# luoyetx/JDA

Measured on AMD Instinct MI355X. Metric: candidate windows/sec, 640x480 batch (jdaDetect hot path); FDDB images/sec in config.fddb_images_per_s, higher is better.
Workload: dtype f32

## Files before the change

### jda_amd/csrc/host.h

```cpp
#pragma once
#include <hip/hip_runtime_api.h>

#include <algorithm>
#include <atomic>
#include <chrono>
#include <cmath>
#include <cstdio>
#include <cstdlib>
#include <cstring>
#include <condition_variable>
#include <exception>
#include <functional>
#include <memory>
#include <map>
#include <mutex>
#include <numeric>
#include <new>
#include <stdexcept>
#include <string>
#include <thread>
#include <tuple>
#include <vector>

#include "../../include/jda.h"
// ... 34 lines not shown
  catch (const std::exception& e) { std::snprintf(buf, sizeof buf, "%s", e.what()); what = buf; }
  catch (...) {}
  try { fail(std::string(fn) + ": " + what); }
  catch (...) { std::fprintf(stderr, "libjda: %s: %s\n", fn, what); }
  if (sync_device) { (void)hipDeviceSynchronize(); (void)hipGetLastError(); }
}
#define JDA_ABI_CATCH(ret) catch (...) { jda::abi_exception(__func__, false); return ret; }
#define JDA_ABI_CATCH_SYNC(ret) catch (...) { jda::abi_exception(__func__, true); return ret; }
#define JDA_ABI_CATCH_VOID catch (...) { jda::abi_exception(__func__, false); }

constexpr int kLdsGranule = 1280, kLdsGranules = 128;
inline int lds_wgs_per_cu(long long lds_bytes) { return lds_bytes <= 0 ? kLdsGranules : (int)(kLdsGranules / ((lds_bytes + kLdsGranule - 1) / kLdsGranule)); }
inline int lds_bytes_for_wgs(int wgs_per_cu) { return (kLdsGranules / std::max(1, wgs_per_cu)) * kLdsGranule; }

inline long long env_ll(const char* name, long long dflt) {
  const char* v = std::getenv(name);
  return v && *v ? std::atoll(v) : dflt;
}

#define JDA_KNOBS(X)                                                                                   \
  X(handoff, "JDA_HANDOFF", 128)             \
  X(no_fast_scan, "JDA_NO_FAST_SCAN", 0)                                                               \
  X(plan_cache, "JDA_PLAN_CACHE", 64)                                 \
  X(dense, "JDA_DENSE", 1)                                                \
  X(merge_blocks, "JDA_MERGE_BLOCKS", 2048)  \
  X(side_small, "JDA_SIDE_SMALL", 1)                                                                   \
  X(side_stream, "JDA_SIDE_STREAM", 1)                                                                 \
  X(wide_max, "JDA_WIDE_MAX", 1024)          \
  X(wide_conc, "JDA_WIDE_CONC", 1)           \
  X(h2d_stream, "JDA_H2D_STREAM", 1)         \
  X(h2d_min_bytes, "JDA_H2D_MIN_BYTES", 8 << 20)  \
  X(kernel_d2h, "JDA_KERNEL_D2H", 1)         \
  X(filter0, "JDA_FILTER0", 1)               \
  X(predict, "JDA_PREDICT", 1)               \
  X(debug_times, "JDA_DEBUG_TIMES", 0)                                                                 \
  X(test_wpf_scale, "JDA_TEST_WPF_SCALE", 1)              \
  X(test_throw, "JDA_TEST_THROW", 0)         \
  X(lanes, "JDA_LANES", 2)                                 \
  X(lanes_min_windows, "JDA_LANES_MIN_WINDOWS", 2000000)                                               \
  X(workspace_mb, "JDA_WORKSPACE_MB", 24 * 1024)                                                       \
  X(ws_bound, "JDA_WS_BOUND", 1)             \
  X(ws_factor_pct, "JDA_WS_FACTOR_PCT", 400)  \
  X(ws_min_entries, "JDA_WS_MIN_ENTRIES", 65536)  \
  X(ragged_chunk_windows, "JDA_RAGGED_CHUNK_WINDOWS", 4000000)  \
  X(ragged_chunk_windows_cpp, "JDA_RAGGED_CHUNK_WINDOWS_CPP", 8000000)  \
  X(mine_chunk_windows, "JDA_MINE_CHUNK_WINDOWS", 4194304)  \
  X(ragged_chunk_min_windows, "JDA_RAGGED_CHUNK_MIN_WINDOWS", 1500000)  \
  X(ragged_split, "JDA_RAGGED_SPLIT", 3)     \
  X(ragged_single_windows, "JDA_RAGGED_SINGLE_WINDOWS", 5000000)  \
  X(hwq_place, "JDA_HWQ_PLACE", 1)           \
  X(max_lanes, "JDA_MAX_LANES", 16)          \
  X(lane_idle_calls, "JDA_LANE_IDLE_CALLS", 256)  \
  X(device_post, "JDA_DEVICE_POST", 1)       \
  X(device_post_min_frames, "JDA_DEVICE_POST_MIN_FRAMES", 16)  \
  X(w_pad, "JDA_W_PAD", 1)                   \
  X(lm_deep, "JDA_LM_DEEP", 1)               \
  X(w_stream_mb, "JDA_W_STREAM_MB", 8)       \
  X(scan_p, "JDA_SCAN_P", 1)                 \
  X(scan_p_ragged, "JDA_SCAN_P_RAGGED", 1)   \
  X(scan_p_block, "JDA_SCAN_P_BLOCK", 768)                               \
  X(scan_p_slots, "JDA_SCAN_P_SLOTS", 5)     \
  X(scan_p_b0, "JDA_SCAN_P_B0", 32)                \
  X(scan_p_b1, "JDA_SCAN_P_B1", 64)                                                                    \
  X(scan_p_b2, "JDA_SCAN_P_B2", 0)                                                                     \
  X(scan_p_b3, "JDA_SCAN_P_B3", 0)                                                                     \
  X(scan_p_b4, "JDA_SCAN_P_B4", 0)                                                                     \
// ... 454 lines not shown
```

### jda_amd/csrc/k_finish.hip

```cpp
#include "finish_common.h"

#ifndef FIN_ROW_BATCH
#define FIN_ROW_BATCH 0
#endif

namespace jda {


template <typename DL, bool TRACE, int kG, bool MULTI, bool ST, bool STREAM = false>
__global__ __launch_bounds__(64) void k_finish(const DevPlan* __restrict__ plan, DevModelT<typename DL::Real> m,
                                               WorkT<typename DL::Real> w, int multi_i, float inv_sqrt2,
                                               int t_begin, int t_end, int apply_th, typename DL::Real final_th,
                                               const S0Node* __restrict__ s0_table, int tile_win, int survivors) {
  using Real = typename DL::Real;
  constexpr bool kCpp = sizeof(Real) == 8;
  extern __shared__ __attribute__((aligned(16))) unsigned char lds[];
  const int lane = threadIdx.x;
  const int T = m.T, K = m.K, node_n = m.node_n, leaf_n = m.leaf_n, dim = m.dim, w_pitch = m.w_pitch;
  const int dim_pad = (dim + 1) & ~1;
  Real* sh = (Real*)lds;
  uint32_t* lbf = (uint32_t*)(sh + dim_pad);
  int* stage_cnt = (int*)(lbf + ((K + 3) & ~3));
  Real* st_tmp = (Real*)(stage_cnt + kMaxStages);
  uint8_t* tile = lds + (((size_t)((unsigned char*)(st_tmp + (ST ? 2 * dim_pad + 8 : 0)) - lds) + 15) & ~(size_t)15);
  constexpr bool multi = MULTI;
  (void)multi_i;
  if (lane < kMaxStages) stage_cnt[lane] = 0;
  const bool from_scan = t_begin == 0 && !survivors;
  const unsigned n = (unsigned)min(w.counters[from_scan ? kCntTail : kCntMid], (unsigned long long)(from_scan ? w.cap_q : w.cap_m));
  unsigned long long carts_acc = 0;

#ifdef JDA_SCAN_TIMING
  unsigned long long stamps[15];
  int n_stamp = 0;
  int dbg_win = 0;
#define JDA_FSTAMP() do { if (n_stamp < 15) stamps[n_stamp++] = __builtin_amdgcn_s_memtime(); } while (0)
#else
#define JDA_FSTAMP() do { } while (0)
#endif
  for (unsigned i = blockIdx.x; i < n; i += gridDim.x) {
    JDA_FSTAMP();
    const uint32_t gid = from_scan ? w.q_gid[i] : w.m_gid[i];
    Real score = from_scan ? w.q_score[i] : w.m_score[i];
    const int kstart = from_scan ? (int)w.q_kstart[i] : (survivors ? K : 0);
    unsigned hash = kFnvSeed;
    if (TRACE) hash = from_scan ? w.q_hash[i] : w.m_hash[i];
    int win;
    View v0{}, v1{}, v2{};
    const uint32_t xy = from_scan ? w.q_xy[i] : w.m_xy[i];
    const uint32_t wf = from_scan ? w.q_wf[i] : w.m_wf[i];
    decode_window<Real>(plan, w, xy, wf, inv_sqrt2, &win, &v0, &v1, &v2, multi);
    const S0Node* s0_tbl = nullptr;
    if (!MULTI && s0_table != nullptr && t_begin == 0) {
      const bool hit = lane < plan->n_levels && plan->lv[lane].win == win;
      const unsigned long long mh = __ballot(hit);
      if (mh) {
        const DevLevel lv = plan->lv[__ffsll((long long)mh) - 1];
        if (lv.tiled) s0_tbl = s0_table + lv.s0_table;
      }
    }
    const uint8_t* wbase = v0.img + (size_t)v0.oy * v0.w + v0.ox;
#ifdef JDA_SCAN_TIMING
    dbg_win = win;
#endif
    const bool use_tile = !MULTI && win <= tile_win;
    const int tpitch = (win + 3) & ~3;
    __syncthreads();
    if (!MULTI && use_tile) load_window_tile(wbase, v0.w, win, tile, tpitch, lane, 64, v0.bc);
    {
      const Real* src = t_begin == 0 ? m.mean_shape : w.m_shape + (size_t)i * dim;
      for (int d = lane; d < dim; d += 64) sh[d] = src[d];
    }
    __syncthreads();
    JDA_FSTAMP();

    bool alive = true;
    int carts_n = 0;
    for (int t = t_begin; t < t_end; t++) {
      const NodeOff<Real>* n_off = (const NodeOff<Real>*)m.lm_off + (size_t)t * K * node_n;
      const uint2* n_meta = m.lm_meta + (size_t)t * K * node_n;
      const int n_split = m.lm_split;
      const typename DL::Node* n_deep = (const typename DL::Node*)m.lm_deep + (size_t)t * K * (node_n - ((1 << min(n_split, m.D - 1)) - 1));
      const Real* leaf_tab = m.leaf + (size_t)t * K * leaf_n;
      const Real* cth = m.cth + (size_t)t * K;
      const Real* cmean = m.cmean + (size_t)t * K;
      const Real* cstd = m.cstd + (size_t)t * K;
      const uint8_t* cnorm = m.cnorm + (size_t)t * K;
      const int kbeg = t == 0 ? min(kstart, K) : 0;
      const int k_first = kbeg & ~63;
      Stp<Real> stp;
      stp.scale = 1; stp.r00 = 1; stp.r01 = 0; stp.r10 = 0; stp.r11 = 1;
      if constexpr (ST) {
        const bool stale = t == m.similarity - 2;
        if (lane == 0 && (!stale || t == t_begin)) {
          Stp<double> p;
          p.scale = 1.; p.r00 = 1.; p.r01 = 0.; p.r10 = 0.; p.r11 = 1.;
          if (!stale) p = stp_calc((const double*)sh, (const double*)m.mean_shape_raw, m.L, (double*)st_tmp, (double*)st_tmp + dim_pad);
          double* o = (double*)st_tmp + 2 * dim_pad;
          o[0] = p.scale; o[1] = p.r00; o[2] = p.r01; o[3] = p.r10; o[4] = p.r11;
        }
        __syncthreads();
        const Real* o = st_tmp + 2 * dim_pad;
        stp.scale = o[0]; stp.r00 = o[1]; stp.r01 = o[2]; stp.r10 = o[3]; stp.r11 = o[4];
      }
      const bool apply_st = ST && t > 0;

      for (int k0 = k_first; k0 < K && alive; k0 += 64 * kG) {
        int kk[kG], lf[kG], nrm[kG];
        Real ls[kG], thk[kG], mk[kG], sk[kG];
#pragma unroll
        for (int g = 0; g < kG; g++) kk[g] = min(k0 + g * 64 + lane, K - 1);
        if (t == 0 && s0_tbl && use_tile) walk_carts_s0<kG, true>(s0_tbl, K, kk, m.D, node_n, tile, tpitch, lf, Bc(0, (long long)tpitch * win));
        else if (t == 0 && s0_tbl) walk_carts_s0<kG, false>(s0_tbl, K, kk, m.D, node_n, wbase, v0.w, lf, v0.bc);
        else if (!MULTI && use_tile) walk_carts<DL, kG, MULTI, ST, true>(n_off, n_meta, K, kk, m.D, node_n, sh, win, v0, v1, v2, stp, apply_st, lf, tile, tpitch, n_deep, n_split);
        else walk_carts<DL, kG, MULTI, ST>(n_off, n_meta, K, kk, m.D, node_n, sh, win, v0, v1, v2, stp, apply_st, lf, nullptr, 0, n_deep, n_split);
#pragma unroll
        for (int g = 0; g < kG; g++) {
          const int k = k0 + g * 64 + lane;
          ls[g] = 0; thk[g] = 0; mk[g] = 0; sk[g] = 1; nrm[g] = 0;
          if (k < K) {
            lbf[k] = (uint32_t)(k * leaf_n + lf[g]) * (uint32_t)w_pitch;
            ls[g] = leaf_tab[(unsigned)(k * leaf_n + lf[g])];
            thk[g] = cth[k];
            nrm[g] = cnorm[k];
            if (nrm[g]) { mk[g] = cmean[k]; sk[g] = cstd[k]; }
          }
        }
#pragma unroll
        for (int g = 0; g < kG; g++) {
          const int kg = k0 + g * 64;
          if (kg >= K || !alive) break;
          const unsigned long long normmask = __ballot(nrm[g] != 0);
          const int jr = replay_scores<Real, TRACE>(score, hash, ls[g], thk[g], mk[g], sk[g], normmask, lf[g],
                                                    max(0, kbeg - kg), min(64, K - kg));
          if (jr >= 0) { alive = false; carts_n = t * K + kg + jr + 1; }
        }
        if (t == t_begin) JDA_FSTAMP();
      }
      if (t != t_begin) JDA_FSTAMP();
      if (!alive) break;
      for (int k0 = 0; k0 < k_first; k0 += 128) {
        int kk[2], lf[2];
        kk[0] = min(k0 + lane, k_first - 1); kk[1] = min(k0 + 64 + lane, k_first - 1);
        if (t == 0 && s0_tbl && use_tile) walk_carts_s0<2, true>(s0_tbl, K, kk, m.D, node_n, tile, tpitch, lf, Bc(0, (long long)tpitch * win));
        else if (t == 0 && s0_tbl) walk_carts_s0<2, false>(s0_tbl, K, kk, m.D, node_n, wbase, v0.w, lf, v0.bc);
        else if (!MULTI && use_tile) walk_carts<DL, 2, MULTI, ST, true>(n_off, n_meta, K, kk, m.D, node_n, sh, win, v0, v1, v2, stp, apply_st, lf, tile, tpitch, n_deep, n_split);
        else walk_carts<DL, 2, MULTI, ST>(n_off, n_meta, K, kk, m.D, node_n, sh, win, v0, v1, v2, stp, apply_st, lf, nullptr, 0, n_deep, n_split);
        if (k0 + lane < k_first) lbf[k0 + lane] = (uint32_t)((k0 + lane) * leaf_n + lf[0]) * (uint32_t)w_pitch;
        if (k0 + 64 + lane < k_first) lbf[k0 + 64 + lane] = (uint32_t)((k0 + 64 + lane) * leaf_n + lf[1]) * (uint32_t)w_pitch;
      }
      __syncthreads();
      if (t == t_begin) JDA_FSTAMP();
      const Real* wt = m.w_rows + (size_t)t * K * leaf_n * w_pitch;
      for (int d = lane; d < dim; d += 64) {
        Real acc = kCpp ? (Real)0 : sh[d];
        const Real* col = wt + d;
        int k = 0;
#ifdef JDA_EXP_NOREG
        k = K;
#endif
        constexpr int RB = FIN_ROW_BATCH > 0 ? FIN_ROW_BATCH : (kCpp ? 32 : 64);
        for (; k + RB <= K; k += RB) {
          Real r[RB];
#pragma unroll
          for (int u = 0; u < RB; u++) { JDA_BC(Bc(0, (long long)K * leaf_n * w_pitch), (long long)lbf[k + u] + d, 1, kBcWRow); r[u] = STREAM ? __builtin_nontemporal_load(col + lbf[k + u]) : col[lbf[k + u]]; }
#pragma unroll
          for (int u = 0; u < RB; u++) acc = acc + r[u];
        }
        for (; k < K; k++) { JDA_BC(Bc(0, (long long)K * leaf_n * w_pitch), (long long)lbf[k] + d, 1, kBcWRow); acc = acc + col[lbf[k]]; }
        if (kCpp) {
          const Real other = __shfl_xor(acc, 1);
          acc = (d & 1) ? stp.scale * (stp.r10 * other + stp.r11 * acc) : stp.scale * (stp.r00 * acc + stp.r01 * other);
          acc = sh[d] + acc;
// ... 49 lines not shown
namespace {
__device__ __forceinline__ int walk_cart_s0_d4(const S0Node* __restrict__ tbl, unsigned K, unsigned k,
                                               const uint8_t* __restrict__ pix, int pitch, const Bc& bc = Bc()) {
  const S0Node r0 = tbl[k];
  const uint4 c1 = *(const uint4*)(tbl + K + 2u * k);
  const uint4 c2a = *(const uint4*)(tbl + 3u * K + 4u * k);
  const uint4 c2b = *(const uint4*)(tbl + 3u * K + 4u * k + 2u);
  auto left = [&](uint32_t lo, uint32_t hi) {
    const unsigned p1 = lo & 0x3fffffu, p2 = __builtin_amdgcn_alignbit(hi, lo, 22) & 0x3fffffu;
    JDA_BC_ADDR(bc, pix + __umul24(p1 >> 11, (unsigned)pitch) + (p1 & 0x7ffu), 1, kBcFinishPix);
    JDA_BC_ADDR(bc, pix + __umul24(p2 >> 11, (unsigned)pitch) + (p2 & 0x7ffu), 1, kBcFinishPix);
    const int a = pix[__umul24(p1 >> 11, (unsigned)pitch) + (p1 & 0x7ffu)];
    const int b = pix[__umul24(p2 >> 11, (unsigned)pitch) + (p2 & 0x7ffu)];
    return a - b <= (int)((hi >> 12) & 0x3ffu) - 256;
  };
  const bool l0 = left(r0.lo, r0.hi);
  const uint32_t lo1 = l0 ? c1.x : c1.z, hi1 = l0 ? c1.y : c1.w;
  const bool l1 = left(lo1, hi1);
  const uint32_t lo2 = l0 ? (l1 ? c2a.x : c2a.z) : (l1 ? c2b.x : c2b.z);
  const uint32_t hi2 = l0 ? (l1 ? c2a.y : c2a.w) : (l1 ? c2b.y : c2b.w);
  const bool l2 = left(lo2, hi2);
  const int n1 = l0 ? 1 : 2, n2 = 2 * n1 + (l1 ? 1 : 2), n3 = 2 * n2 + (l2 ? 1 : 2);
  return n3 - 7;
}
}

template <typename DL, bool TRACE>
__global__ __launch_bounds__(256) void k_filter0(const DevPlan* __restrict__ plan, DevModelT<typename DL::Real> m,
                                                 WorkT<typename DL::Real> w, const S0Node* __restrict__ s0_table) {
  using Real = typename DL::Real;
  constexpr int NW = 2;
  const int lane = threadIdx.x & 63, wv = threadIdx.x >> 6;
  const int K = m.K, node_n = m.node_n, leaf_n = m.leaf_n;
  const unsigned n = (unsigned)min(w.counters[kCntTail], (unsigned long long)w.cap_q);
  const Real* leaf_tab = m.leaf;
  const int W = plan->width;
#ifdef JDA_BOUNDS_CHECK
  const Bc bc_fr((long long)(uintptr_t)w.bc_lo, (long long)(uintptr_t)w.bc_hi);
#else
  const Bc bc_fr;
#endif
  unsigned long long carts_acc = 0;
  const unsigned waves = gridDim.x * 4u;
  for (unsigned i0 = blockIdx.x * 4u + (unsigned)wv; i0 < n; i0 += NW * waves) {
    unsigned idx[NW]; bool has[NW];
    uint32_t gid[NW], xy[NW], wf[NW];
    Real score[NW];
    int kbeg[NW], rej[NW];
    unsigned hash[NW];
    const uint8_t* wbase[NW];
    const S0Node* tbl[NW];
#pragma unroll
    for (int u = 0; u < NW; u++) {
      idx[u] = i0 + (unsigned)u * waves; has[u] = idx[u] < n;
      const unsigned i = has[u] ? idx[u] : i0;
      gid[u] = w.q_gid[i]; score[u] = w.q_score[i]; kbeg[u] = min((int)w.q_kstart[i], K);
      hash[u] = TRACE ? w.q_hash[i] : kFnvSeed;
      xy[u] = w.q_xy[i]; wf[u] = w.q_wf[i];
      rej[u] = has[u] ? -1 : 0;
    }
#pragma unroll
    for (int u = 0; u < NW; u++) {
      const int win = (int)(wf[u] & 0xffffu), frame = (int)(wf[u] >> 16);
      const uint8_t* img = w.img_off != nullptr ? w.frames + w.img_off[frame] : w.frames + (size_t)frame * w.frame_stride;
      wbase[u] = img + (size_t)(xy[u] >> 16) * W + (xy[u] & 0xffffu);
      tbl[u] = s0_table;
      const bool hit = lane < plan->n_levels && plan->lv[lane].win == win;
      const unsigned long long mh = __ballot(hit);
      if (mh) tbl[u] = s0_table + plan->lv[__ffsll((long long)mh) - 1].s0_table;
    }
    int k0[NW];
#pragma unroll
    for (int u = 0; u < NW; u++) k0[u] = kbeg[u] & ~63;
    for (;;) {
      bool go[NW], any = false;
#pragma unroll
      for (int u = 0; u < NW; u++) { go[u] = rej[u] < 0 && k0[u] < K; any = any || go[u]; }
      if (!any) break;
      int lf[NW], nrm[NW];
      Real ls[NW], thk[NW], mk[NW], sk[NW];
#pragma unroll
      for (int u = 0; u < NW; u++) {
        const int k = k0[u] + lane;
        thk[u] = 0; nrm[u] = 0; ls[u] = 0; mk[u] = 0; sk[u] = 1; lf[u] = 0;
        if (go[u] && k < K) { thk[u] = m.cth[k]; nrm[u] = m.cnorm[k]; }
      }
#pragma unroll
      for (int u = 0; u < NW; u++) {
        if (!go[u]) continue;
        int kk[1], l1[1];
        kk[0] = min(k0[u] + lane, K - 1);
        if (m.D == 4) l1[0] = walk_cart_s0_d4(tbl[u], (unsigned)K, (unsigned)kk[0], wbase[u], W, bc_fr);
        else walk_carts_s0<1, false>(tbl[u], K, kk, m.D, node_n, wbase[u], W, l1, bc_fr);
        lf[u] = l1[0];
      }
#pragma unroll
      for (int u = 0; u < NW; u++) {
        const int k = k0[u] + lane;
        if (go[u] && k < K) {
          ls[u] = leaf_tab[(unsigned)(k * leaf_n + lf[u])];
          if (nrm[u]) { mk[u] = m.cmean[k]; sk[u] = m.cstd[k]; }
        }
      }
#pragma unroll
      for (int u = 0; u < NW; u++) {
        if (!go[u]) continue;
        const unsigned long long normmask = __ballot(nrm[u] != 0);
        const int jr = replay_scores<Real, TRACE>(score[u], hash[u], ls[u], thk[u], mk[u], sk[u], normmask, lf[u],
                                                  max(0, kbeg[u] - k0[u]), min(64, K - k0[u]));
        if (jr >= 0) rej[u] = k0[u] + jr;
        k0[u] += 64;
      }
    }
#pragma unroll
    for (int u = 0; u < NW; u++) {
      if (!has[u]) continue;
      if (rej[u] >= 0) {
        carts_acc += (unsigned long long)(rej[u] + 1);
        if (TRACE && lane == 0) { w.tr_carts[gid[u]] = rej[u] + 1; w.tr_score[gid[u]] = score[u]; w.tr_hash[gid[u]] = hash[u]; }
      } else {
        unsigned o = 0;
        if (lane == 0) o = (unsigned)atomicAdd(&w.counters[kCntMid], 1ull);
        o = (unsigned)__shfl((int)o, 0);
        if (o < w.cap_m && lane == 0) {
          w.m_gid[o] = gid[u]; w.m_score[o] = score[u]; w.m_xy[o] = xy[u]; w.m_wf[o] = wf[u];
          if (TRACE) w.m_hash[o] = hash[u];
        }
      }
    }
  }
  if (lane == 0 && carts_acc) atomicAdd(shard_counter(w.counters, kCntCarts), carts_acc);
}

template <typename Real>
hipError_t launch_filter0(bool trace, const DevPlan* d_plan, const DevModelT<Real>& m, const WorkT<Real>& w, long long n_hint,
                          const S0Node* s0_table, hipStream_t stream) {
  using DL = typename std::conditional<sizeof(Real) == 4, DialectC, DialectCPP>::type;
  const unsigned blocks = (unsigned)std::max<long long>(1, std::min<long long>((n_hint + 7) / 8, 1 << 20));
  if (trace) hipLaunchKernelGGL((k_filter0<DL, true>), dim3(blocks), dim3(256), 0, stream, d_plan, m, w, s0_table);
  else hipLaunchKernelGGL((k_filter0<DL, false>), dim3(blocks), dim3(256), 0, stream, d_plan, m, w, s0_table);
  return hipGetLastError();
}
template hipError_t launch_filter0<float>(bool, const DevPlan*, const DevModelT<float>&, const WorkT<float>&, long long, const S0Node*, hipStream_t);
template hipError_t launch_filter0<double>(bool, const DevPlan*, const DevModelT<double>&, const WorkT<double>&, long long, const S0Node*, hipStream_t);

namespace {
template <typename DL>
hipError_t launch_finish_impl(bool trace, int t_begin, int t_end, bool apply_th, typename DL::Real th,
                              const DevPlan* d_plan, const DevModelT<typename DL::Real>& m,
                              const WorkT<typename DL::Real>& w, int groups, long long n_hint, const S0Node* s0_table,
                              int tile_win, bool survivors, hipStream_t stream) {
  using Real = typename DL::Real;
  const int dim_pad = (m.dim + 1) & ~1;
  const bool st = sizeof(Real) == 8 && m.similarity != 0;
  const int multi = (w.half != nullptr) ? 1 : 0;
  if (multi) tile_win = 0;
  const size_t base = (size_t)dim_pad * sizeof(Real) + (size_t)((m.K + 3) & ~3) * 4 + kMaxStages * sizeof(int) +
                      (st ? (2 * (size_t)dim_pad + 8) * sizeof(Real) : 0);
  if (tile_win < 0) {
// ... 62 lines not shown
```

### jda_amd/csrc/k_scan_p.hip

```cpp
#include "kernels_common.h"
#include "scan_walk.h"

namespace jda {

namespace {

constexpr int kPSlotsMax = 8;
constexpr int kPWidxBits = 11;
constexpr int kPBaseBits = 18;
constexpr int kPSpinMax = 1 << 20;
#ifndef JDA_SCAN_P_IDLE_MAX
#define JDA_SCAN_P_IDLE_MAX (1 << 20)
#endif
constexpr int kPIdleMax = JDA_SCAN_P_IDLE_MAX;

struct ThNormF { float th, norm; };

typedef int v4i __attribute__((ext_vector_type(4)));
struct PCtl {
  v4i rec[32];
  int cfgw[64];
  unsigned long long dbg[20];
};
constexpr int kRecRing = 8, kRecMisc = 14, kRecGeo = 16, kRecGeo2 = 24;
// ... 299 lines not shown
      if (lane == 0) atomicOr(scan_err, 2ull);
      return true;
    }
    if (lane == 0) st_relaxed(rw, start + n);
    JDA_PSUB_END(8);
    return true;
  };
  auto hand_off = [&](bool alive, uint32_t packed, float score) {
    const unsigned long long mask = __ballot(alive);
    const int n = __popcll(mask);
    if (n == 0) return;
    unsigned gbase = 0;
    if (lane == 0) gbase = (unsigned)atomicAdd(&w.counters[cfg.to_mid ? kCntMid : kCntTail], (unsigned long long)n);
    gbase = (unsigned)uni((int)gbase);
    if (alive) {
      const int rank = __popcll(mask & lanes_below(lane));
      const int s = (int)(packed >> (kPBaseBits + kPWidxBits));
      const int widx = (int)((packed >> kPBaseBits) & ((1u << kPWidxBits) - 1u));
      const v4i g = rec_l[kRecGeo + s];
      v4i g2 = g;
      if (RAGGED) g2 = rec_l[kRecGeo2 + s];
      const int tw_s = RAGGED ? g2.z : lv.tw;
      const int wy = widx / tw_s, wx = widx - wy * tw_s;
      const int frame = g.z, wx0 = g.w & 0xffff, wy0 = (int)((unsigned)g.w >> 16);
      const unsigned slot = gbase + (unsigned)rank;
      if (slot < (cfg.to_mid ? w.cap_m : w.cap_q)) {
        JDA_BC(Bc(0, cfg.to_mid ? w.cap_m : w.cap_q), slot, 1, kBcQueue);
        const uint32_t gid = RAGGED ? (uint32_t)(g2.x + (wy0 + wy) * g2.y + wx0 + wx)
                                    : (uint32_t)(frame * plan->windows + lv.base + (wy0 + wy) * lv.nx + wx0 + wx);
        const uint32_t xy = (uint32_t)((wx0 + wx) * lv.step) | ((uint32_t)((wy0 + wy) * lv.step) << 16);
        const uint32_t wf = (uint32_t)lv.win | ((uint32_t)frame << 16);
        if (cfg.to_mid) {
          w.m_gid[slot] = gid; w.m_score[slot] = score; w.m_xy[slot] = xy; w.m_wf[slot] = wf;
        } else {
          w.q_gid[slot] = gid; w.q_score[slot] = score; w.q_kstart[slot] = (uint32_t)K; w.q_xy[slot] = xy; w.q_wf[slot] = wf;
        }
      }
      handed += K;
      if (cfg.to_mid) mids += 1;
    }
    lds_drain();
  };
  int rv = -2;
  uint32_t r_pk = 0u;
  float r_sc = 0.f;
  bool r_ok = false;

  const unsigned slot_bits = (1u << S) - 1u;
  for (;;) {
    if (rv == -2) {
      {
        const v4i r = rec_l[lane & 15];
        compiler_fence();
        const bool is_slot = lane < S, is_ring = (unsigned)(lane - kRecRing) < (unsigned)NB;
        const int bidx = r.y & 0xfff;
        const int avail_v = r.x - r.y;
        const int sx = r.x & 3;
        const unsigned m_dr = (unsigned)__ballot(is_slot && (sx == 0 || (sx == 2 && bidx >= r.z && r.w == 0)));
        const unsigned m_fr = (unsigned)__ballot(is_slot && sx == 2 && bidx < r.z);
        const unsigned m_full = (unsigned)__ballot(is_ring && avail_v >= need_v);
        const int next_j = __builtin_amdgcn_readlane(r.x, kRecMisc);
        int task = -1;
        int t_b = 0, t_n = 0, t_s = 0, t_j = 0, t_gen = 0, t_xg = 0;
        uint2 t_it = make_uint2(0u, 0u);
        bool lost = false;
        unsigned m_ring = m_full;
// ... 261 lines not shown
```

### jda_amd/csrc/kernels.h

```cpp
#pragma once
#include <hip/hip_runtime_api.h>

#include <cstddef>
#include <cstdint>

namespace jda {

constexpr int kMaxLevels = 64;
constexpr int kMaxStages = 16;

struct DevLevel {
  int win, step, nx, ny;
  int base;
  int tiled;
  int tw, th;
  int tiles_x, tiles_y;
  int pitch;
  int s0_table;
};

struct DevPlan {
  int n_levels;
  int width, height;
  int windows;
// ... 55 lines not shown
template <typename Real>
struct DevModelT {
  int T, K, L, D, node_n, leaf_n, dim;
  const void* nodes;
  const void* lm_off;
  const uint2* lm_meta;
  const void* lm_deep;
  int lm_split;
  const Real* leaf;
  const Real* cth;
  const Real* cmean;
  const Real* cstd;
  const uint8_t* cnorm;
  const void* par0;
  const Real* w;
  const Real* w_rows;
  int w_pitch;
  int w_stream;
  const Real* mean_shape;
  const Real* mean_shape_raw;
  int similarity;
};

template <typename Real>
struct WorkT {
  const uint8_t* frames; size_t frame_stride; int n_frames;
  const uint8_t* half; size_t half_stride; int hw, hh;
  const uint8_t* quarter; size_t quarter_stride; int qw, qh;
  int patch_hs, patch_qs;
  uint32_t* q_gid; Real* q_score; uint32_t* q_hash; uint32_t* q_kstart;
  uint32_t* q_xy; uint32_t* q_wf;
  unsigned long long* counters;
  uint32_t* m_gid; Real* m_score; uint32_t* m_hash; Real* m_shape; uint32_t* m_xy; uint32_t* m_wf;
  int* st_carts;
  uint32_t* out_gid; Real* out_score; Real* out_shape;
  int* tr_carts; Real* tr_score; uint32_t* tr_hash; Real* tr_shape;
  unsigned cap;
  unsigned cap_q, cap_m;
  const RagSeg* segs; const RagBlk* blk; const unsigned long long* img_off;
#ifdef JDA_SCAN_TIMING
  unsigned long long* dbg;
#endif
#ifdef JDA_BOUNDS_CHECK
  const uint8_t* bc_lo; const uint8_t* bc_hi;
#endif
};

constexpr int kCntShards = 64;
constexpr int kCntStride = 32;

enum Counter : int {
  kCntStage0 = 0,
  kCntTail = kMaxStages,
  kCntOut = kMaxStages + 1,
  kCntCarts = kMaxStages + 2,
  kCntCartsScan = kMaxStages + 3,
  kCntWinScan = kMaxStages + 4,
  kCntMid = kMaxStages + 5,
  kCntCartsScanGlb = kMaxStages + 6,
  kCntTotal = kMaxStages + 7,
  kCntMidScan = kCntStride - 1,
  kCntPostCursor = kCntTotal,
  kCntScanErr = kCntTotal
};
constexpr int kCntScanErrShard = 9;
static_assert(kCntTotal <= kCntStride, "counter shard too small");


hipError_t launch_resize(const uint8_t* src, size_t src_stride, int n, int sw, int sh,
                         uint8_t* dst, size_t dst_stride, int dw, int dh, float rx, float ry,
                         hipStream_t stream);

hipError_t launch_resize_cv(const uint8_t* src, size_t src_stride, int n, int sw, int sh,
                            uint8_t* dst, size_t dst_stride, int dw, int dh, hipStream_t stream);

hipError_t launch_resize_cv_patches(const uint8_t* src, size_t src_stride, int n, int lw, int nx, int ny, int step, int win,
                                    uint8_t* dst, size_t dst_stride, int ds, hipStream_t stream);

hipError_t launch_prep_stage0(int dialect, const DevPlan* d_plan, const DevPlan& h_plan,
// ... 126 lines not shown
```

### jda_amd/csrc/lanes.cpp

```cpp
#include "host.h"

namespace jda {


namespace {
constexpr long long kSpinBase = 20000, kSpinStep = 5000;
}

int StreamPool::classify(hipStream_t s) {
  const int m = (int)rep.size();
  if (m == 0) return -1;
  if (!stamps) {
    if (hipHostMalloc((void**)&stamps, sizeof(unsigned long long) * kSlots * kRow, hipHostMallocDefault) != hipSuccess) { (void)hipGetLastError(); stamps = nullptr; return -3; }
    std::memset(stamps, 0, sizeof(unsigned long long) * kSlots * kRow);
  }
  volatile unsigned long long* h = stamps + (size_t)(probe_no++ % kSlots) * kRow;
  for (int k = 0; k <= m; k++) h[k] = 0;
  for (int k = 0; k < m; k++)
    if (launch_hwq_spin(kSpinBase + k * kSpinStep, (unsigned long long*)(h + k), rep[k]) != hipSuccess) return -3;
  if (launch_hwq_stamp((unsigned long long*)(h + m), s) != hipSuccess || hipStreamSynchronize(s) != hipSuccess) return -3;
  probes++;
  const unsigned long long t = h[m];
  int best = -1;
  unsigned long long best_d = ~0ull;
// ... 110 lines not shown
  return true;
}

Lane* acquire_lane_locked(Cascador* c, size_t want_cap, bool* exhausted, Lane::Bag* trimmed) {
  Lane* best = nullptr;
  for (auto& up : c->lanes) {
    Lane* l = up.get();
    if (l->busy) continue;
    if (!best) { best = l; continue; }
    const bool fit = l->cap >= want_cap, bfit = best->cap >= want_cap;
    if (fit != bfit ? fit : (fit ? l->cap < best->cap : l->cap > best->cap)) best = l;
  }
  if (!best) {
    if ((long long)c->lanes.size() >= std::max<long long>(1, c->kn.max_lanes)) { if (exhausted) *exhausted = true; return nullptr; }
    std::unique_ptr<Lane> l(new (std::nothrow) Lane());
    if (!l || !l->create(&c->streams)) { if (l) l->destroy(); return nullptr; }
    best = l.get();
    c->lanes.push_back(std::move(l));
  }
  const long long idle_max = c->kn.lane_idle_calls;
  for (auto& up : c->lanes) {
    Lane* l = up.get();
    if (l->busy || l == best) continue;
    if (idle_max > 0 && ++l->idle > (unsigned long long)idle_max && (l->ws.p || l->frames.p || l->rag_frames.p)) l->trim(trimmed);
  }
  best->busy = true;
  best->idle = 0;
  return best;
}


template <typename Real>
size_t bytes_per_window(int dim, bool trace) {
  size_t b = (4 + sizeof(Real) + 4 + 8) + 2 * (4 + sizeof(Real) + (size_t)dim * sizeof(Real)) + 8 + 4;
  if (trace) b += 4 + 4 + sizeof(Real) + 4 + (size_t)dim * sizeof(Real);
  return b;
}

namespace {
template <typename Real>
size_t carve_workspace(void* base, WorkT<Real>& w, size_t cap, size_t cap_q, size_t cap_m, bool trace, bool dense, int dim) {
  Carver cv(base);
  w.q_gid = cv.take<uint32_t>(cap_q);
  w.q_score = cv.take<Real>(cap_q);
  w.q_kstart = cv.take<uint32_t>(cap_q);
  w.q_xy = cv.take<uint32_t>(cap_q);
  w.q_wf = cv.take<uint32_t>(cap_q);
  w.q_hash = trace ? cv.take<uint32_t>(cap_q) : nullptr;
  w.m_gid = cv.take<uint32_t>(cap_m);
  w.m_score = cv.take<Real>(cap_m);
  w.m_hash = trace ? cv.take<uint32_t>(cap_m) : nullptr;
  w.m_shape = cv.take<Real>(cap_m * dim);
  w.m_xy = cv.take<uint32_t>(cap_m);
  w.m_wf = cv.take<uint32_t>(cap_m);
  w.st_carts = dense ? cv.take<int>(cap) : nullptr;
  w.out_gid = cv.take<uint32_t>(cap_m);
  w.out_score = cv.take<Real>(cap_m);
  w.out_shape = cv.take<Real>(cap_m * dim);
  w.counters = cv.take<unsigned long long>(kCntShards * kCntStride);
#ifdef JDA_SCAN_TIMING
  w.dbg = cv.take<unsigned long long>(65536 * 32);
#endif
  if (trace) {
    w.tr_carts = cv.take<int>(cap); w.tr_score = cv.take<Real>(cap);
    w.tr_hash = cv.take<uint32_t>(cap); w.tr_shape = cv.take<Real>(cap * dim);
  } else {
    w.tr_carts = nullptr; w.tr_score = nullptr; w.tr_hash = nullptr; w.tr_shape = nullptr;
  }
  return cv.off + 256;
}
}

template <typename Real>
size_t workspace_bytes(size_t cap, size_t cap_q, size_t cap_m, bool trace, bool dense, int dim) {
  WorkT<Real> w{};
  if (dense) cap_m = std::max(cap_m, cap);
  return carve_workspace<Real>(nullptr, w, cap, std::min(cap_q, cap), std::min(cap_m, cap), trace, dense, dim);
}

template <typename Real>
bool ensure_workspace(Lane* ln, size_t cap, bool trace, int dim, size_t cap_q, size_t cap_m, bool dense) {
  if (cap_q == 0 || cap_q > cap) cap_q = cap;
  if (cap_m == 0 || cap_m > cap) cap_m = cap;
  if (dense) cap_m = cap;
  const bool same = ln->dim == dim && ln->real_bytes == (int)sizeof(Real);
  if (same && ln->cap >= cap && ln->cap_q >= cap_q && ln->cap_m >= cap_m && (ln->trace || !trace) && (ln->dense_ws || !dense)) return true;
  if (same) {
// ... 46 lines not shown
```

### jda_amd/csrc/pass.h

```cpp
#pragma once
#include "host.h"

namespace jda {

inline int scan_p_base_cfg(const Cascador* c, PScanCfg* cfg, int* block, int* wgs) {
  const Knobs& kn = c->kn;
  const int K = std::min(c->hm.K, (int)(kn.scan_p_handoff > 0 ? kn.scan_p_handoff : kn.handoff));
  const long long bs[5] = {kn.scan_p_b0, kn.scan_p_b1, kn.scan_p_b2, kn.scan_p_b3, kn.scan_p_b4};
  int digits[kPScanMaxBuckets] = {6, 6, 6, 6, 6, 6}, nd = 0;
  { long long v = std::max<long long>(0, kn.scan_p_lg); int tmp[16]; int n = 0; while (v > 0 && n < 16) { tmp[n++] = (int)(v % 10); v /= 10; }
    for (int i = n - 1; i >= 0 && nd < kPScanMaxBuckets; i--) digits[nd++] = tmp[i]; }
  int last = 0;
  for (int i = 0; i < 5 && cfg->nb < kPScanMaxBuckets; i++) {
    const int b = (int)bs[i];
    if (b <= last || b >= K) continue;
    cfg->bound[cfg->nb] = b;
    const int d = digits[cfg->nb];
    cfg->lg[cfg->nb] = ((d == 4 || d == 5 || d == 7 || d == 8 || d == 9) && c->hm.leaf_n() <= 256) || d == 2 || d == 3 ? d : 6;
    cfg->nb++;
    last = b;
  }
  cfg->bound[cfg->nb] = K;
  cfg->bound_last = K;
  cfg->any_norm = stage0_any_norm(c->hm, K, true) ? 1 : 0;
// ... 68 lines not shown
  }
  int f0 = 0, nf = 0;
  const unsigned char* const* host_frames = nullptr; size_t host_fbytes = 0;
  const RaggedChunk* rag = nullptr;
  bool dense = false, finished = false, lds_span = false;
  bool timed = true;
  bool predicted = false;
  bool counters_issued = false, results_pending = false;
  int p_launches = 0;
  bool want_post = false, post_nms = true; float post_overlap = 0.3f;
  bool post_issued = false, posted = false; size_t post_cap = 0;
  bool mid_direct = false;
  bool no_scan_p = false;
  int my_scan_launches = 0;
  uint8_t* a_hbuf = nullptr; size_t a_hs = 0; uint8_t* a_qbuf = nullptr; size_t a_qs = 0;
  long long n_tail = -1;
  size_t n_out = 0, out_copied = 0;

  const HostModel& hm() const { return c->hm; }
  const DevModelT<Real>& model() const { return Sel<Real>::model(c).m; }
  bool want_trace() const { return trace != nullptr; }
  int stage_groups() const {
    const int K = hm().K;
    int best = 4, best_waste = 1 << 30;
    for (int g = 4; g >= 2; g--) {
      const int per = 64 * g, waste = ((K + per - 1) / per) * per - K;
      if (waste < best_waste) { best = g; best_waste = waste; }
    }
    return best;
  }
  const S0Node* s0_tbl() const { return (pe->fast_scan && pe->table && pe->lm_ok && c->kn.fin_s0) ? pe->table + pe->table_cap : nullptr; }
  const Knobs& kn() const { return c->kn; }
  bool filter0_ok() const { return kn().filter0 && s0_tbl() != nullptr && pe->fast_scan && !pe->any_untiled && !multi; }
  long long windows() const { return rag ? rag->windows : (long long)nf * pe->sp.windows; }

  bool dense_ok(int* pix_cap, int* lds_max) const {
    constexpr int dialect = Sel<Real>::dialect;
    const long long dense_env = kn().dense;
    *lds_max = (int)kn().dense_lds_max;
    const int dim = hm().dim();
    const int fixed = (int)stage_lds_bytes(dim, hm().node_n(), hm().leaf_n(), (int)sizeof(Real));
    *pix_cap = std::max(0, std::min<int>((int)kn().dense_pix, *lds_max - fixed));
    return dense_env != 0 && !multi && !(dialect == JDA_DIALECT_CPP && c->similarity) &&
           dim <= 160 && hm().leaf_n() <= 256 && fixed <= *lds_max;
  }
  bool run_dense() {
    int pix_cap, lds_max;
    (void)dense_ok(&pix_cap, &lds_max);
    for (int t = 0; t < hm().T; t++)
      for (int l = 0; l < pe->hp.n_levels; l++)
        JDA_HIP(launch_stage<Real>(want_trace(), l, t, apply_th, th, pe->dp, pe->hp, model(), w, pix_cap, lds_max, st));
    return true;
  }
  bool clear_counters() {
    JDA_HIP(hipMemsetAsync(w.counters, 0, sizeof(unsigned long long) * kCntShards * kCntStride, st));
    if (want_trace()) {
      JDA_HIP(hipMemsetAsync(w.tr_carts, 0, sizeof(int) * (size_t)windows(), st));
      JDA_HIP(launch_trace_fill<Real>(model(), w, (unsigned)windows(), st));
    }
    return true;
  }
  bool read_counter(int counter) {
    const size_t n = counter == kCntTail ? (size_t)(kCntMid - kCntTail + 1) : 1;
    JDA_HIP(hipMemcpyAsync(h_cnt, w.counters + counter, n * sizeof(unsigned long long), hipMemcpyDeviceToHost, st));
    return true;
  }
// ... 244 lines not shown
      JDA_HIP(hipStreamWaitEvent(ln->side, ln->ev_side[0], 0));
    }
    auto issue = [&](const RaggedChunk::Launch& l, hipStream_t s, bool try_persistent) -> bool {
      if (try_persistent && l.mode == 1 && l.level >= 0 && scan_persistent(l.level, s, &l)) { rs->scan_launches++; my_scan_launches++; return true; }
      JDA_HIP(launch_scan_ragged<Real>(l.mode, l.block, false, handoff, cp_max, opts, pe->dp, m, pe->table, w, l.pix_bytes,
                                       l.blk_base, l.blk_n, s));
      rs->scan_launches++; my_scan_launches++;
      return true;
    };
    if (fork_glb) {
      for (const RaggedChunk::Launch& l : ch.launches)
        if (l.mode == 2) { if (!issue(l, ln->side, false)) return false; side_pending = true; }
    }
    for (const RaggedChunk::Launch& l : ch.launches) {
      if (l.mode == 2 && fork_glb) continue;
      if (fork_glb && kn().ragged_side == 2 && l.mode != 2) {
        if (l.mode == 1 && l.level >= 0 && scan_persistent(l.level, st, &l)) { rs->scan_launches++; my_scan_launches++; continue; }
        if (!issue(l, ln->side, false)) return false;
        continue;
      }
      if (!issue(l, st, true)) return false;
    }
    if (side_pending) JDA_HIP(hipEventRecord(ln->ev_side[1], ln->side));
    if (side_pending) JDA_HIP(hipStreamWaitEvent(st, ln->ev_side[1], 0));
    if (timed) JDA_HIP(hipEventRecord(ev[2], st));
    return issue_rest();
  }

  bool launch_finishers(long long n_grid) {
    const int T = hm().T;
    const int gm = kn().fin_gm > 0 ? (int)kn().fin_gm : stage_groups();
    const int g2 = kn().fin_g2 > 0 ? (int)kn().fin_g2 : stage_groups();
    n_grid = std::max<long long>(n_grid, 1);
    if (mid_direct) {
      const long long nmid = pred_mid >= 0 ? (long long)(pred_mid * (double)windows() * 1.25) + 64 : 0;
      const long long wg2 = std::min<long long>((long long)cap_m, std::max<long long>(std::max<long long>(2048, n_grid / std::max<long long>(1, kn().fin_grid_div)), nmid));
      JDA_HIP(launch_filter0<Real>(want_trace(), pe->dp, model(), w, n_grid, s0_tbl(), st));
      JDA_HIP(launch_finish<Real>(want_trace(), 0, T, apply_th, th, pe->dp, model(), w, g2, wg2, s0_tbl(), (int)kn().fin_tile, st, true));
      finished = true;
      return true;
    }
    if (n_grid <= kn().wide_max && busy_lanes <= kn().wide_busy_max && finish_wide_ok(hm().dim(), hm().K, hm().leaf_n(), (int)sizeof(Real), multi, Sel<Real>::dialect == JDA_DIALECT_CPP && c->similarity)) {
      JDA_HIP(launch_finish_wide<Real>(want_trace(), apply_th, th, pe->dp, model(), w, n_grid, s0_tbl(), st, kn().wide_conc != 0));
      finished = true;
      return true;
    }
    const bool st_snapshot = sizeof(Real) == 8 && c->similarity && hm().hdr_stage >= 0 && hm().hdr_stage < T;
    if (T == 1 || n_grid <= kn().finish_merge || st_snapshot) {
      JDA_HIP(launch_finish<Real>(want_trace(), 0, T, apply_th, th, pe->dp, model(), w, gm, n_grid, s0_tbl(), (int)kn().fin_tile, st));
      finished = true;
      return true;
    }
    const long long wg2 = std::min<long long>(n_grid, std::max<long long>(2048, n_grid / std::max<long long>(1, kn().fin_grid_div)));
    if (filter0_ok()) {
      JDA_HIP(launch_filter0<Real>(want_trace(), pe->dp, model(), w, n_grid, s0_tbl(), st));
      JDA_HIP(launch_finish<Real>(want_trace(), 0, T, apply_th, th, pe->dp, model(), w, g2, wg2, s0_tbl(), (int)kn().fin_tile, st, true));
      finished = true;
      return true;
    }
    JDA_HIP(launch_finish<Real>(want_trace(), 0, 1, apply_th, th, pe->dp, model(), w, (int)kn().fin_g1, n_grid, s0_tbl(), (int)kn().fin_tile1, st));
    JDA_HIP(launch_finish<Real>(want_trace(), 1, T, apply_th, th, pe->dp, model(), w, g2, wg2, nullptr, (int)kn().fin_tile, st));
    finished = true;
    return true;
  }

  bool after_tail() {
    if (finished) return true;
    JDA_HIP(hipStreamSynchronize(st));
    const unsigned long long true_tail = h_cnt[0], true_mid = mid_direct ? h_cnt[kCntMid - kCntTail] : 0ull;
    n_tail = (long long)std::min<unsigned long long>(true_tail, cap_q);
    const long long n_alive = (long long)(true_tail + true_mid);
    int pix_cap, lds_max;
    const double dense_frac = (double)kn().dense_pct / 100.0;
    if (dense_ok(&pix_cap, &lds_max) && (double)n_alive >= dense_frac * (double)windows() && n_alive > 4096) {
      { std::lock_guard<std::mutex> lk(c->mu); pe->dense_hint = true; }
      if (!rag) {
        dense = true; finished = true;
        if (!grow_for_dense() || !clear_counters()) return false;
        return run_dense();
      }
    }
    if (true_tail > cap_q || true_mid > cap_m) return recover_overflow(true_tail, true_mid, 0);
    return launch_finishers(n_tail);
  }

  bool after_mid() { return true; }

  bool issue_counters() {
    if (counters_issued) return true;
// ... 243 lines not shown
```

Measured before the change: 7.313 billion.

## Carry stage-0 leaf indices from filter0 into finish to skip re-walking carts

filter0 now packs each lane's stage-0 leaf index per 64-cart round into a 32-bit word and stores it, along with the starting round, for surviving windows. k_finish reads these packed leaves for the carried rounds and fills the leaf-offset buffer directly instead of re-walking the stage-0 trees. This removes the duplicated tree walks in the finish kernel. In exchange it adds workspace (64 words per window, capped at 65536 windows), extra global writes in filter0, and only applies when leaf bits times rounds fit in 32 bits.

```diff
diff --git a/jda_amd/csrc/host.h b/jda_amd/csrc/host.h
--- a/jda_amd/csrc/host.h
+++ b/jda_amd/csrc/host.h
@@ -90,6 +90,7 @@
   X(h2d_min_bytes, "JDA_H2D_MIN_BYTES", 8 << 20)  \
   X(kernel_d2h, "JDA_KERNEL_D2H", 1)         \
   X(filter0, "JDA_FILTER0", 1)               \
+  X(fin_carry, "JDA_FIN_CARRY", 1)           \
   X(predict, "JDA_PREDICT", 1)               \
   X(debug_times, "JDA_DEBUG_TIMES", 0)                                                                 \
   X(test_wpf_scale, "JDA_TEST_WPF_SCALE", 1)              \
diff --git a/jda_amd/csrc/k_finish.hip b/jda_amd/csrc/k_finish.hip
--- a/jda_amd/csrc/k_finish.hip
+++ b/jda_amd/csrc/k_finish.hip
@@ -43,6 +43,7 @@
     const uint32_t gid = from_scan ? w.q_gid[i] : w.m_gid[i];
     Real score = from_scan ? w.q_score[i] : w.m_score[i];
     const int kstart = from_scan ? (int)w.q_kstart[i] : (survivors ? K : 0);
+    const int kc = survivors && w.m_leaf != nullptr ? min((int)w.m_k0[i], K) : K;
     unsigned hash = kFnvSeed;
     if (TRACE) hash = from_scan ? w.q_hash[i] : w.m_hash[i];
     int win;
@@ -87,7 +88,8 @@
       const Real* cstd = m.cstd + (size_t)t * K;
       const uint8_t* cnorm = m.cnorm + (size_t)t * K;
       const int kbeg = t == 0 ? min(kstart, K) : 0;
-      const int k_first = kbeg & ~63;
+      const bool carried = t == 0 && kc < K;
+      const int k_first = carried ? kc : kbeg & ~63;
       Stp<Real> stp;
       stp.scale = 1; stp.r00 = 1; stp.r01 = 0; stp.r10 = 0; stp.r11 = 1;
       if constexpr (ST) {
@@ -105,7 +107,7 @@
       }
       const bool apply_st = ST && t > 0;
 
-      for (int k0 = k_first; k0 < K && alive; k0 += 64 * kG) {
+      for (int k0 = carried ? K : k_first; k0 < K && alive; k0 += 64 * kG) {
         int kk[kG], lf[kG], nrm[kG];
         Real ls[kG], thk[kG], mk[kG], sk[kG];
 #pragma unroll
@@ -139,6 +141,13 @@
       }
       if (t != t_begin) JDA_FSTAMP();
       if (!alive) break;
+      if (carried) {
+        const int bits = carry_bits(leaf_n);
+        const uint32_t word = w.m_leaf[(size_t)i * 64 + lane];
+        for (int k = kc + lane; k < K; k += 64)
+          lbf[k] = (uint32_t)(k * leaf_n + carry_unpack(word, bits, k >> 6)) * (uint32_t)w_pitch;
+        JDA_FSTAMP();
+      }
       for (int k0 = 0; k0 < k_first; k0 += 128) {
         int kk[2], lf[2];
         kk[0] = min(k0 + lane, k_first - 1); kk[1] = min(k0 + 64 + lane, k_first - 1);
@@ -254,6 +263,8 @@
   constexpr int NW = 2;
   const int lane = threadIdx.x & 63, wv = threadIdx.x >> 6;
   const int K = m.K, node_n = m.node_n, leaf_n = m.leaf_n;
+  const bool carry = w.m_leaf != nullptr;
+  const int cbits = carry_bits(leaf_n);
   const unsigned n = (unsigned)min(w.counters[kCntTail], (unsigned long long)w.cap_q);
   const Real* leaf_tab = m.leaf;
   const int W = plan->width;
@@ -266,7 +277,7 @@
   const unsigned waves = gridDim.x * 4u;
   for (unsigned i0 = blockIdx.x * 4u + (unsigned)wv; i0 < n; i0 += NW * waves) {
     unsigned idx[NW]; bool has[NW];
-    uint32_t gid[NW], xy[NW], wf[NW];
+    uint32_t gid[NW], xy[NW], wf[NW], packed[NW];
     Real score[NW];
     int kbeg[NW], rej[NW];
     unsigned hash[NW];
@@ -274,7 +285,7 @@
     const S0Node* tbl[NW];
 #pragma unroll
     for (int u = 0; u < NW; u++) {
-      idx[u] = i0 + (unsigned)u * waves; has[u] = idx[u] < n;
+      idx[u] = i0 + (unsigned)u * waves; has[u] = idx[u] < n; packed[u] = 0u;
       const unsigned i = has[u] ? idx[u] : i0;
       gid[u] = w.q_gid[i]; score[u] = w.q_score[i]; kbeg[u] = min((int)w.q_kstart[i], K);
       hash[u] = TRACE ? w.q_hash[i] : kFnvSeed;
@@ -315,6 +326,7 @@
         if (m.D == 4) l1[0] = walk_cart_s0_d4(tbl[u], (unsigned)K, (unsigned)kk[0], wbase[u], W, bc_fr);
         else walk_carts_s0<1, false>(tbl[u], K, kk, m.D, node_n, wbase[u], W, l1, bc_fr);
         lf[u] = l1[0];
+        if (carry) packed[u] = carry_pack(packed[u], lf[u], cbits, k0[u] >> 6);
       }
 #pragma unroll
       for (int u = 0; u < NW; u++) {
@@ -347,6 +359,11 @@
         if (o < w.cap_m && lane == 0) {
           w.m_gid[o] = gid[u]; w.m_score[o] = score[u]; w.m_xy[o] = xy[u]; w.m_wf[o] = wf[u];
           if (TRACE) w.m_hash[o] = hash[u];
+        }
+        if (carry && o < w.cap_m) {
+          const bool room = o < w.cap_l && kbeg[u] < K;
+          if (room) w.m_leaf[(size_t)o * 64 + lane] = packed[u];
+          if (lane == 0) w.m_k0[o] = room ? (uint32_t)(kbeg[u] & ~63) : (uint32_t)K;
         }
       }
     }
diff --git a/jda_amd/csrc/k_scan_p.hip b/jda_amd/csrc/k_scan_p.hip
--- a/jda_amd/csrc/k_scan_p.hip
+++ b/jda_amd/csrc/k_scan_p.hip
@@ -355,6 +355,7 @@
         const uint32_t wf = (uint32_t)lv.win | ((uint32_t)frame << 16);
         if (cfg.to_mid) {
           w.m_gid[slot] = gid; w.m_score[slot] = score; w.m_xy[slot] = xy; w.m_wf[slot] = wf;
+          w.m_k0[slot] = (uint32_t)K;
         } else {
           w.q_gid[slot] = gid; w.q_score[slot] = score; w.q_kstart[slot] = (uint32_t)K; w.q_xy[slot] = xy; w.q_wf[slot] = wf;
         }
diff --git a/jda_amd/csrc/kernels.h b/jda_amd/csrc/kernels.h
--- a/jda_amd/csrc/kernels.h
+++ b/jda_amd/csrc/kernels.h
@@ -111,6 +111,7 @@
   uint32_t* q_xy; uint32_t* q_wf;
   unsigned long long* counters;
   uint32_t* m_gid; Real* m_score; uint32_t* m_hash; Real* m_shape; uint32_t* m_xy; uint32_t* m_wf;
+  uint32_t* m_leaf; uint32_t* m_k0; unsigned cap_l;
   int* st_carts;
   uint32_t* out_gid; Real* out_score; Real* out_shape;
   int* tr_carts; Real* tr_score; uint32_t* tr_hash; Real* tr_shape;
@@ -124,6 +125,31 @@
   const uint8_t* bc_lo; const uint8_t* bc_hi;
 #endif
 };
+
+constexpr unsigned kCarryCapMax = 1u << 16;
+__host__ __device__ constexpr int carry_bits(int leaf_n) { int b = 0; while ((1 << b) < leaf_n) b++; return b; }
+__host__ __device__ constexpr int carry_rounds(int K) { return (K + 63) >> 6; }
+__host__ __device__ constexpr bool carry_fits(int leaf_n, int K) { return carry_bits(leaf_n) * carry_rounds(K) <= 32; }
+__host__ __device__ constexpr uint32_t carry_pack(uint32_t word, int leaf, int bits, int round) { return word | ((uint32_t)leaf << (bits * round)); }
+__host__ __device__ constexpr int carry_unpack(uint32_t word, int bits, int round) { return (int)((word >> (bits * round)) & ((1u << bits) - 1u)); }
+namespace carry_check {
+__host__ __device__ constexpr bool round_trip(int leaf_n, int K) {
+  const int bits = carry_bits(leaf_n), rounds = carry_rounds(K);
+  if (!carry_fits(leaf_n, K)) return false;
+  for (int seed = 0; seed < leaf_n; seed++) {
+    uint32_t word = 0;
+    for (int r = 0; r < rounds; r++) word = carry_pack(word, (seed + r * 5) % leaf_n, bits, r);
+    for (int r = 0; r < rounds; r++) if (carry_unpack(word, bits, r) != (seed + r * 5) % leaf_n) return false;
+  }
+  return true;
+}
+static_assert(carry_bits(2) == 1 && carry_bits(4) == 2 && carry_bits(8) == 3 && carry_bits(1) == 0 && carry_bits(32) == 5, "bits = ceil(log2(leaf_n))");
+static_assert(carry_rounds(64) == 1 && carry_rounds(540) == 9 && carry_rounds(682) == 11, "rounds = ceil(K / 64)");
+static_assert(round_trip(2, 64) && round_trip(4, 64) && round_trip(8, 64), "K = 64");
+static_assert(round_trip(2, 540) && round_trip(4, 540) && round_trip(8, 540), "K = 540: 27 bits with depth-4 trees");
+static_assert(round_trip(2, 682) && round_trip(4, 682) && !carry_fits(8, 682), "K = 682: 11 rounds, depth 4 needs 33 bits -- no carry");
+static_assert(!carry_fits(32, 2000) && carry_fits(2, 2048) && !carry_fits(2, 2049), "depth 6 with K = 2000 walks as before; 32 rounds of one bit fit");
+}
 
 constexpr int kCntShards = 64;
 constexpr int kCntStride = 32;
diff --git a/jda_amd/csrc/lanes.cpp b/jda_amd/csrc/lanes.cpp
--- a/jda_amd/csrc/lanes.cpp
+++ b/jda_amd/csrc/lanes.cpp
@@ -166,7 +166,7 @@
 
 template <typename Real>
 size_t bytes_per_window(int dim, bool trace) {
-  size_t b = (4 + sizeof(Real) + 4 + 8) + 2 * (4 + sizeof(Real) + (size_t)dim * sizeof(Real)) + 8 + 4;
+  size_t b = (4 + sizeof(Real) + 4 + 8) + 2 * (4 + sizeof(Real) + (size_t)dim * sizeof(Real)) + 8 + 4 + 4;
   if (trace) b += 4 + 4 + sizeof(Real) + 4 + (size_t)dim * sizeof(Real);
   return b;
 }
@@ -187,6 +187,9 @@
   w.m_shape = cv.take<Real>(cap_m * dim);
   w.m_xy = cv.take<uint32_t>(cap_m);
   w.m_wf = cv.take<uint32_t>(cap_m);
+  w.m_k0 = cv.take<uint32_t>(cap_m);
+  w.cap_l = (unsigned)std::min<size_t>(cap_m, kCarryCapMax);
+  w.m_leaf = cv.take<uint32_t>((size_t)w.cap_l * 64);
   w.st_carts = dense ? cv.take<int>(cap) : nullptr;
   w.out_gid = cv.take<uint32_t>(cap_m);
   w.out_score = cv.take<Real>(cap_m);
diff --git a/jda_amd/csrc/pass.h b/jda_amd/csrc/pass.h
--- a/jda_amd/csrc/pass.h
+++ b/jda_amd/csrc/pass.h
@@ -124,6 +124,7 @@
   const S0Node* s0_tbl() const { return (pe->fast_scan && pe->table && pe->lm_ok && c->kn.fin_s0) ? pe->table + pe->table_cap : nullptr; }
   const Knobs& kn() const { return c->kn; }
   bool filter0_ok() const { return kn().filter0 && s0_tbl() != nullptr && pe->fast_scan && !pe->any_untiled && !multi; }
+  bool carry_ok() const { return kn().fin_carry && filter0_ok() && carry_fits(hm().leaf_n(), hm().K); }
   long long windows() const { return rag ? rag->windows : (long long)nf * pe->sp.windows; }
 
   bool dense_ok(int* pix_cap, int* lds_max) const {
@@ -434,11 +435,13 @@
     const int gm = kn().fin_gm > 0 ? (int)kn().fin_gm : stage_groups();
     const int g2 = kn().fin_g2 > 0 ? (int)kn().fin_g2 : stage_groups();
     n_grid = std::max<long long>(n_grid, 1);
+    WorkT<Real> wc = w;
+    if (!carry_ok()) wc.m_leaf = nullptr;
     if (mid_direct) {
       const long long nmid = pred_mid >= 0 ? (long long)(pred_mid * (double)windows() * 1.25) + 64 : 0;
       const long long wg2 = std::min<long long>((long long)cap_m, std::max<long long>(std::max<long long>(2048, n_grid / std::max<long long>(1, kn().fin_grid_div)), nmid));
-      JDA_HIP(launch_filter0<Real>(want_trace(), pe->dp, model(), w, n_grid, s0_tbl(), st));
-      JDA_HIP(launch_finish<Real>(want_trace(), 0, T, apply_th, th, pe->dp, model(), w, g2, wg2, s0_tbl(), (int)kn().fin_tile, st, true));
+      JDA_HIP(launch_filter0<Real>(want_trace(), pe->dp, model(), wc, n_grid, s0_tbl(), st));
+      JDA_HIP(launch_finish<Real>(want_trace(), 0, T, apply_th, th, pe->dp, model(), wc, g2, wg2, s0_tbl(), (int)kn().fin_tile, st, true));
       finished = true;
       return true;
     }
@@ -455,8 +458,8 @@
     }
     const long long wg2 = std::min<long long>(n_grid, std::max<long long>(2048, n_grid / std::max<long long>(1, kn().fin_grid_div)));
     if (filter0_ok()) {
-      JDA_HIP(launch_filter0<Real>(want_trace(), pe->dp, model(), w, n_grid, s0_tbl(), st));
-      JDA_HIP(launch_finish<Real>(want_trace(), 0, T, apply_th, th, pe->dp, model(), w, g2, wg2, s0_tbl(), (int)kn().fin_tile, st, true));
+      JDA_HIP(launch_filter0<Real>(want_trace(), pe->dp, model(), wc, n_grid, s0_tbl(), st));
+      JDA_HIP(launch_finish<Real>(want_trace(), 0, T, apply_th, th, pe->dp, model(), wc, g2, wg2, s0_tbl(), (int)kn().fin_tile, st, true));
       finished = true;
       return true;
     }
```

After: 7.396 billion (median of 6 runs). 1.1% higher.
